# Project-Splinter/MonoPort

Measured on AMD Instinct MI355X. Metric: reconstructions/sec (512^2 in, 256^3 grid), higher is better.
Workload: dtype f32

## Files before the change

### monoport_amd/csrc/api.hip

```cpp
#include <cstdarg>
#include <cmath>
#include <cstring>

#include "mp_internal.h"
#include "encoder_kernels.h"
#include "octree_common.h"

namespace mp {

static thread_local std::string g_last_error;

int fail(mp_ctx *ctx, int code, const char *fmt, ...) {
  (void)ctx;
  char buf[512];
  va_list ap;
  va_start(ap, fmt);
  vsnprintf(buf, sizeof(buf), fmt, ap);
  va_end(ap);
  g_last_error = buf;
  return code;
}

int ensure_scratch(mp_ctx *ctx, hipStream_t st, size_t bytes, void **out) {
  mp_ctx::Arena &a = ctx->arenas[(void *)st];
// ... 2357 lines not shown
  DeviceGuard g(ctx->device);
  return launch_conv3x3_wino_pack(ctx, w, cout, cin, packed_wino, (hipStream_t)stream);
}

int mp_conv3x3_wino_supported(int cin, int cout, int h, int w) { return conv3x3_wino_supported(cin, cout, h, w) ? 1 : 0; }

int mp_conv3x3_pack16(mp_ctx *ctx, const float *w, int cout, int cin, void *packed16, float *wmax,
                      mp_stream stream) {
  if (!ctx) return MP_ERR_ARG;
  std::lock_guard<std::mutex> lk(ctx->mu);
  if (!w || !packed16 || !wmax || cout <= 0 || cin <= 0)
    return fail(ctx, MP_ERR_ARG, "mp_conv3x3_pack16: bad argument");
  if (cin % 16 || cout % 32)
    return fail(ctx, MP_ERR_UNSUPPORTED, "mp_conv3x3_pack16: needs Cin %% 16 == 0 and Cout %% 32 == 0");
  DeviceGuard g(ctx->device);
  return launch_conv3x3_pack16(ctx, w, cout, cin, packed16, wmax, (hipStream_t)stream);
}

int mp_conv3x3_gn16(mp_ctx *ctx, const float *x, int n, int cin, int h, int w, const float *ss, int relu,
                    int reflect, const void *packed16, const float *wmax, int cout, float *y, double *stats,
                    mp_stream stream) {
  if (!ctx) return MP_ERR_ARG;
  std::lock_guard<std::mutex> lk(ctx->mu);
  if (!x || !packed16 || !wmax || !y || n <= 0 || n > 65535 || cin <= 0 || cout <= 0 || h <= 0 || w <= 0)
    return fail(ctx, MP_ERR_ARG, "mp_conv3x3_gn16: bad argument");
  if (!aligned16(packed16)) return fail(ctx, MP_ERR_ARG, "mp_conv3x3_gn16: packed weights must be 16-byte aligned");
  DeviceGuard g(ctx->device);
  return launch_conv3x3_gn(ctx, x, n, cin, h, w, ss, relu, reflect, static_cast<const float *>(packed16),
                           wmax, cout, y, stats, (hipStream_t)stream);
}

int mp_conv1x1_pack(mp_ctx *ctx, const float *w1, int c1, const float *w2, int c2, int cout, int f16,
                    void *packed, float *wmax, mp_stream stream) {
  if (!ctx) return MP_ERR_ARG;
  std::lock_guard<std::mutex> lk(ctx->mu);
  if (!w1 || !packed || c1 <= 0 || c2 < 0 || (c2 > 0 && !w2) || (f16 && !wmax))
    return fail(ctx, MP_ERR_ARG, "mp_conv1x1_pack: bad argument");
  if (c1 % 64 || c2 % 64 || (cout != 128 && cout != 256))
    return fail(ctx, MP_ERR_UNSUPPORTED,
                "mp_conv1x1_pack: input channel counts must be multiples of 64, output channels 128 or 256");
  DeviceGuard g(ctx->device);
  return launch_conv1x1_pack(ctx, w1, c1, w2, c2, cout, f16, packed, wmax, (hipStream_t)stream);
}

int mp_conv1x1(mp_ctx *ctx, const float *x1, const float *ss1, int relu1, const float *x2, int n, int c1,
               int c2, int cout, int64_t hw, const void *packed, int f16, const float *wmax, const float *bias,
               const float *res, float *y, float *y_hwc, double *stats, mp_stream stream) {
  if (!ctx) return MP_ERR_ARG;
  std::lock_guard<std::mutex> lk(ctx->mu);
  if (!x1 || !packed || n <= 0 || hw <= 0 || (!y && !y_hwc) || (f16 && !wmax))
    return fail(ctx, MP_ERR_ARG, "mp_conv1x1: bad argument");
  if (!aligned16(packed) || (y_hwc && !aligned16(y_hwc)))
    return fail(ctx, MP_ERR_ARG, "mp_conv1x1: packed weights / y_hwc must be 16-byte aligned");
  DeviceGuard g(ctx->device);
  return launch_conv1x1_raw(ctx, x1, ss1, relu1, x2, n, c1, c2, cout, hw, packed, f16, wmax, bias, res, y,
                            y_hwc, stats, (hipStream_t)stream);
}

int mp_scale_shift_add(mp_ctx *ctx, const float *t, const float *ss, const float *res, int n, int c,
                       int64_t hw, float *y, mp_stream stream) {
  if (!ctx) return MP_ERR_ARG;
  std::lock_guard<std::mutex> lk(ctx->mu);
  if (!t || !ss || !res || !y || n <= 0 || c <= 0 || hw <= 0)
    return fail(ctx, MP_ERR_ARG, "mp_scale_shift_add: bad argument");
  if (hw % 4 || !aligned16(t) || !aligned16(res) || !aligned16(y))
    return fail(ctx, MP_ERR_UNSUPPORTED, "mp_scale_shift_add: needs HW %% 4 == 0 and 16-byte aligned buffers");
  DeviceGuard g(ctx->device);
  return launch_scale_shift_add(ctx, t, ss, res, (long long)n * c, hw, y, (hipStream_t)stream);
}

int mp_conv3x3_supported(int cin, int cout, int h, int w) { return conv3x3_supported(cin, cout, h, w) ? 1 : 0; }
int mp_conv_stats_supported(int cout) { return conv_stats_supported(cout) ? 1 : 0; }

int mp_gn_stat_slices(void) { return gn_stat_slices(); }

int mp_conv3x3_stat_slices(int cout, int n, int h, int w, int f16) {
  if (cout < 32 || cout % 32 || n < 1 || h < 1 || w < 32) return 0;
  return conv3x3_stat_slices(cout, n, h, w, f16 != 0);
}

void mp_query_tune(int small_tiles) { mp::query_small_set_gate(small_tiles); }

void mp_conv3x3_tune(int nr) {
  conv3x3_set_nr(nr & 0x1fff);
  conv1x1_set_mrw((nr >> 12) & 3);
}

int mp_conv3x3_gn(mp_ctx *ctx, const float *x, int n, int cin, int h, int w, const float *ss, int relu,
                  int reflect, const float *packed, int cout, float *y, double *stats, mp_stream stream) {
  if (!ctx) return MP_ERR_ARG;
  std::lock_guard<std::mutex> lk(ctx->mu);
  if (!x || !packed || !y || n <= 0 || n > 65535 || cin <= 0 || cout <= 0 || h <= 0 || w <= 0)
    return fail(ctx, MP_ERR_ARG, "mp_conv3x3_gn: bad argument");
  if (!aligned16(packed)) return fail(ctx, MP_ERR_ARG, "mp_conv3x3_gn: packed weights must be 16-byte aligned");
  DeviceGuard g(ctx->device);
  return launch_conv3x3_gn(ctx, x, n, cin, h, w, ss, relu, reflect, packed, nullptr, cout, y, stats,
                           (hipStream_t)stream);
}

int mp_gn_stats(mp_ctx *ctx, const float *x, int n, int c, int64_t hw, int groups, double *partial,
                mp_stream stream) {
  if (!ctx) return MP_ERR_ARG;
  std::lock_guard<std::mutex> lk(ctx->mu);
  if (!x || !partial || n <= 0 || c <= 0 || hw <= 0 || groups <= 0)
    return fail(ctx, MP_ERR_ARG, "mp_gn_stats: bad argument");
  if (c % groups || hw % 4 || !aligned16(x))
    return fail(ctx, MP_ERR_UNSUPPORTED, "mp_gn_stats: needs C %% groups == 0, HW %% 4 == 0, 16-byte aligned x");
  DeviceGuard g(ctx->device);
  return launch_gn_stats(ctx, x, n, c, hw, groups, partial, (hipStream_t)stream);
}

int mp_gn_finalize(mp_ctx *ctx, const double *partial, int n, int c, int groups, int slices,
                   int64_t count, const float *gamma, const float *beta, float eps, float *ss,
                   mp_stream stream) {
  if (!ctx) return MP_ERR_ARG;
  std::lock_guard<std::mutex> lk(ctx->mu);
  if (!partial || !gamma || !beta || !ss || n <= 0 || c <= 0 || groups <= 0 || slices <= 0 ||
      count <= 0 || c % groups || c / groups > 64)
    return fail(ctx, MP_ERR_ARG, "mp_gn_finalize: bad argument");
  DeviceGuard g(ctx->device);
  return launch_gn_finalize(ctx, partial, n, c, groups, slices, (double)count, gamma, beta, eps, ss,
                            (hipStream_t)stream);
}

static GnOut to_out(const mp_gn_out *f) {
  GnOut g = gn_out_none();
  if (!f) return g;
  g.acc = reinterpret_cast<long long *>(f->acc);
  g.partial = f->partial;
  return g;
}
static long long out_cap(const mp_gn_out *f) { return f && f->partial ? (long long)f->partial_doubles : -1; }
static GnIn to_in(const mp_gn_in *f) {
  GnIn g = gn_in_none();
  if (!f) return g;
  g.acc = reinterpret_cast<const long long *>(f->acc);
  g.gamma = f->gamma;
  g.beta = f->beta;
  g.eps = f->eps;
  g.ss = f->acc ? nullptr : f->ss;
  return g;
}

int mp_conv3x3_ex(mp_ctx *ctx, const mp_conv3x3_args *q, mp_stream stream) {
  if (!ctx) return MP_ERR_ARG;
  std::lock_guard<std::mutex> lk(ctx->mu);
  if (!q || !q->x || !q->packed || (!q->y && !q->y2) || q->n <= 0 || q->n > 65535 || q->cin <= 0 || q->cout <= 0 ||
      q->h <= 0 || q->w <= 0)
    return fail(ctx, MP_ERR_ARG, "mp_conv3x3_ex: bad argument");
  if (!aligned16(q->packed)) return fail(ctx, MP_ERR_ARG, "mp_conv3x3_ex: packed weights must be 16-byte aligned");
  DeviceGuard g(ctx->device);
  ConvArgs a;
  a.x = q->x;
  a.gn = to_in(&q->gn);
  a.wp = static_cast<const float *>(q->packed);
  a.y = q->y;
  a.y2 = q->y2;
  a.res = q->res;
  a.y2_c = q->y2 ? q->y2_channels : 32;
  a.y2_off = q->y2 ? q->y2_offset : 0;
  a.fin = to_out(&q->fin);
  a.fin2 = to_out(&q->fin2);
  a.n_img = q->n;
  a.cin = q->cin;
  a.cout = q->cout;
  a.h = q->h;
  a.w = q->w;
// ... 187 lines not shown
```

### monoport_amd/csrc/conv3x3.hip

```cpp
#include "mp_internal.h"
#include "query_common.h"
#include "gn_tail.h"

namespace mp {

constexpr int kCK = 16;
constexpr int kPixBytes = kCK * 4;
constexpr int kMaxCin = 512;
constexpr int kConvWps = 2;
constexpr int kTileW = 32;
constexpr int halo_pixels(int px) { return (px / kTileW + 2) * (kTileW + 2); }
constexpr int stage_iters(int px) { return (halo_pixels(px) + 63) / 64; }

__global__ void conv3x3_pack_kernel(const float *__restrict__ w, int cout, int cin,
                                    float *__restrict__ wp) {
  const long long total = (long long)cout * cin * 9;
  const int kgt = (cin / kCK) * 18;
  for (long long t = blockIdx.x * (long long)blockDim.x + threadIdx.x; t < total;
       t += (long long)gridDim.x * blockDim.x) {
    const int i = (int)(t & 3), lane = (int)((t >> 2) & 63);
    const long long q = t >> 8;
    const int kg = (int)(q % kgt), rb = (int)(q / kgt);
    const int g = kg & 1, tap = (kg >> 1) % 9, chunk = (kg >> 1) / 9;
    const int co = 32 * rb + (lane & 31);
// ... 669 lines not shown
#pragma unroll
  for (int n = 0; n < NR; ++n)
#pragma unroll
    for (int t = 0; t < 16; ++t) v[n][t] = acc[n][t] * inv_scale;
  conv_epilogue<32 * RBW, CW, NR, 16>(p, v, 0, img, tile, tiles, y0, x0, rbi, cwi, lane, smem);
}

__global__ __launch_bounds__(64) void gn_finalize_kernel(const double *__restrict__ partial, int groups,
                                                         int slices, double count, int cpg,
                                                         const float *__restrict__ gamma,
                                                         const float *__restrict__ beta, float eps,
                                                         float *__restrict__ ss) {
  const int g = blockIdx.x % groups, n = blockIdx.x / groups;
  const double *pp = partial + (long long)blockIdx.x * slices * 2;
  double a = 0.0, b = 0.0;
  for (int i = threadIdx.x; i < slices; i += 64) {
    a += pp[2 * i];
    b += pp[2 * i + 1];
  }
#pragma unroll
  for (int o = 32; o > 0; o >>= 1) {
    a += __shfl_xor(a, o);
    b += __shfl_xor(b, o);
  }
  const double mean_d = a / count;
  const double var_d = fmax(b / count - mean_d * mean_d, 0.0);
  const float mean = (float)mean_d;
  const float rstd = (float)(1.0 / sqrt(var_d + (double)eps));
  if ((int)threadIdx.x < cpg) {
    const int c = g * cpg + threadIdx.x;
    const float sc = rstd * gamma[c];
    float *o = ss + ((long long)n * groups * cpg + c) * 2;
    o[0] = sc;
    o[1] = beta[c] - mean * sc;
  }
}

__global__ __launch_bounds__(256) void scale_shift_add_kernel(const float *__restrict__ t,
                                                              const float *__restrict__ ss,
                                                              const float *__restrict__ res,
                                                              long long hw4, long long total4,
                                                              float *__restrict__ y) {
  const f32x4 *t4 = reinterpret_cast<const f32x4 *>(t), *r4 = reinterpret_cast<const f32x4 *>(res);
  f32x4 *y4 = reinterpret_cast<f32x4 *>(y);
  for (long long i = blockIdx.x * (long long)blockDim.x + threadIdx.x; i < total4;
       i += (long long)gridDim.x * blockDim.x) {
    const long long plane = i / hw4;
    const float sc = ss[2 * plane], sh = ss[2 * plane + 1];
    const f32x4 a = t4[i], r = r4[i];
    f32x4 o;
#pragma unroll
    for (int k = 0; k < 4; ++k) o[k] = r[k] + (a[k] * sc + sh);
    y4[i] = o;
  }
}

int launch_scale_shift_add(mp_ctx *ctx, const float *t, const float *ss, const float *res, long long planes,
                           long long hw, float *y, hipStream_t st) {
  const long long total4 = planes * (hw / 4);
  long long blocks = (total4 + 255) / 256;
  if (blocks > 16384) blocks = 16384;
  hipLaunchKernelGGL(scale_shift_add_kernel, dim3((unsigned)blocks), dim3(256), 0, st, t, ss, res, hw / 4,
                     total4, y);
  MP_HIP(ctx, hipGetLastError());
  return MP_OK;
}

int launch_conv3x3_pack(mp_ctx *ctx, const float *w, int cout, int cin, float *wp, hipStream_t st) {
  const long long total = (long long)cout * cin * 9;
  long long blocks = (total + 255) / 256;
  if (blocks > 4096) blocks = 4096;
  hipLaunchKernelGGL(conv3x3_pack_kernel, dim3((unsigned)blocks), dim3(256), 0, st, w, cout, cin, wp);
  MP_HIP(ctx, hipGetLastError());
  return MP_OK;
}

static int g_conv_nr = 0;
static int g_conv_sk = -1;

static int g_conv_wino = 1;
static long long g_conv_wino_min_wgs = 128;

void conv3x3_set_nr(int nr) {
  conv3x3_wino_set_variant((nr & 0x800) ? 64 : (nr & 0x1000) ? 128 : 0);
  nr &= ~0x1800;
  g_conv_nr = nr & 0xff;
  g_conv_wino = (nr >> 8) == 0 ? 1 : 0;
  nr &= ~0x400;
  g_conv_sk = (nr >> 8) == 0 ? -1 : (nr >> 8) - 1;
}

struct ConvPlan {
  int rbw, nr, tw, th, tiles;
  bool sk;
};

static ConvPlan conv_plan(int cout, int n, int h, int w, bool f16) {
  ConvPlan c;
  c.rbw = cout % 128 == 0 ? 4 : cout % 64 == 0 ? 2 : 1;
  const int cw = 4 / c.rbw;
  const long long pix = (long long)n * h * w;
  const long long wg1 = pix / (32 * cw) * (cout / (32 * c.rbw));
  const long long wg2 = wg1 / 2;
  c.nr = ((wg2 + 255) / 256) * 2 <= (wg1 + 255) / 256 ? 2 : 1;
  if (g_conv_nr > 0) c.nr = g_conv_nr;
  if (c.nr > 2 && (c.rbw == 1 || !f16)) c.nr = 2;
  c.sk = !f16 && (g_conv_sk >= 0 ? g_conv_sk == 1 : wg1 < 512);
  if (c.sk) {
    c.rbw = 1;
    c.nr = g_conv_nr > 0 ? (g_conv_nr > 2 ? 2 : g_conv_nr) : (pix / 64 * (cout / 32) >= 512 ? 2 : 1);
    if (h < c.nr) c.nr = 1;
    c.tw = kTileW;
    c.th = c.nr;
  } else {
    c.tw = kTileW;
    c.th = 32 * c.nr * cw / c.tw;
  }
  c.tiles = (h / c.th) * (w / c.tw);
  return c;
}

int conv3x3_stat_slices(int cout, int n, int h, int w, bool f16) { return conv_plan(cout, n, h, w, f16).tiles; }

bool conv3x3_supported(int cin, int cout, int h, int w) {
  return !(cin % kCK || cout % 32 || cin < kCK || cout < 32 || w < 32 || (w & (w - 1)) || h < 8 ||
           (h & (h - 1)));
}

bool conv_stats_supported(int cout) { return cout >= 32 && cout % 32 == 0 && 32 % (cout / 32) == 0; }

int launch_absmax(mp_ctx *ctx, const float *src, long long n, unsigned int *out_bits, hipStream_t st);

int launch_conv3x3_pack16(mp_ctx *ctx, const float *w, int cout, int cin, void *wp, float *wmax,
                          hipStream_t st) {
  const long long total = (long long)cout * cin * 9;
  int rc = launch_absmax(ctx, w, total, reinterpret_cast<unsigned int *>(wmax), st);
  if (rc != MP_OK) return rc;
  long long blocks = (total + 255) / 256;
  if (blocks > 4096) blocks = 4096;
  hipLaunchKernelGGL(conv3x3_pack16_kernel, dim3((unsigned)blocks), dim3(256), 0, st, w, cout, cin, wmax,
                     static_cast<_Float16 *>(wp));
  MP_HIP(ctx, hipGetLastError());
  return MP_OK;
}

template <int RBW, int NR>
static int launch_conv16_t(mp_ctx *ctx, const ConvArgs &a, const float *wmax, int tiles, hipStream_t st) {
  const int lds = 2 * (a.th + 2) * (a.tw + 2) * kPixBytes;
  auto kern = conv3x3_gn16_kernel<RBW, NR>;
  int rc = raise_lds_limit(ctx, reinterpret_cast<const void *>(kern), 2 * halo_pixels(32 * NR * (4 / RBW)) * kPixBytes);
  if (rc != MP_OK) return rc;
  hipLaunchKernelGGL(kern, dim3((unsigned)(tiles * a.n_img), (unsigned)(a.cout / (32 * RBW))), dim3(256),
                     lds, st, a, wmax);
  MP_HIP(ctx, hipGetLastError());
  return MP_OK;
}

template <int RBW, int NR>
static int launch_conv_t(mp_ctx *ctx, const ConvArgs &a, int tiles, hipStream_t st) {
  const int lds = 2 * (a.th + 2) * (a.tw + 2) * kPixBytes;
  auto kern = conv3x3_gn_kernel<RBW, NR>;
  int rc = raise_lds_limit(ctx, reinterpret_cast<const void *>(kern), 2 * halo_pixels(32 * NR * (4 / RBW)) * kPixBytes);
  if (rc != MP_OK) return rc;
  hipLaunchKernelGGL(kern, dim3((unsigned)(tiles * a.n_img), (unsigned)(a.cout / (32 * RBW))), dim3(256),
                     lds, st, a);
  MP_HIP(ctx, hipGetLastError());
  return MP_OK;
}
// ... 531 lines not shown
```

### monoport_amd/csrc/conv_wino.hip

```cpp
#include "mp_internal.h"
#include "query_common.h"
#include "gn_tail.h"

#pragma clang fp contract(off)

namespace mp {

constexpr int kWnThreads = 512;
constexpr int kWnTX = 8, kWnTY = 4;
constexpr int kWnPW = 2 * kWnTX + 2;
constexpr int kWnPH = 2 * kWnTY + 2;
constexpr int kWnPix = kWnPW * kWnPH;
constexpr int kWnPasses = (kWnPix + 63) / 64;
constexpr int kWnRow = 80;
constexpr int kWnRawBytes = kWnPix * kWnRow;
constexpr int kWnVBytes = 16 * 32 * kWnRow;
constexpr int kWnRaw = 0;
constexpr int kWnV = 2 * kWnRawBytes;
constexpr int kWnXchBytes = 8 * 2 * 2 * 4 * 64 * 16;
constexpr int kWnStat = kWnXchBytes;
constexpr int kWnLds = kWnStat + 8192;
constexpr int kWnAhead = 3;
static_assert(kWnV + 2 * kWnVBytes <= kWnXchBytes, "the exchange region covers the K loop's buffers");
static_assert(kWnLds <= 160 * 1024, "LDS");
// ... 464 lines not shown
    ring[i] = wload128(ws, a_base + ((cc >> 1) * 8 + i * 2 + (cc & 1)) * 64);
  };

  stage_load(0);
  GnAffine affine;
  gn_affine_load(p.gn, p.cin, affine);
  gn_load_stats(p.gn, img, gn_stats);
  a_load(0, 0);
  a_load(1, 0);
  __syncthreads();
  gn_table_fill(p.gn, img, p.cin, gn_stats, affine, ss_in);
  __syncthreads();
  stage_store(0);
  stage_load(1);
  __syncthreads();
  transform(0);
  stage_store(1);
  stage_load(2);
  __syncthreads();

#pragma unroll 1
  for (int chunk = 0; chunk < n_chunks; ++chunk) {
    const unsigned char *vb = smem + kW8V + (chunk & 1) * kW8VBytes + boff;
    const bool more1 = chunk + 1 < n_chunks;
    f32x4 b[2];
#pragma unroll
    for (int i = 0; i < 2; ++i) b[i] = *reinterpret_cast<const f32x4 *>(vb + i * 4 * 32 * kW8Row);
    a_load(2, chunk);
    a_load(3, chunk);
    if (more1 && rbh == 0) transform((chunk + 1) & 1);
    __builtin_amdgcn_sched_barrier(0);
#pragma unroll
    for (int ii = 0; ii < 4; ++ii)
#pragma unroll
      for (int i = 0; i < 2; ++i) acc[i] = __builtin_amdgcn_mfma_f32_32x32x2f32(ring[i][ii], b[i][ii], acc[i], 0, 0, 0);
    __builtin_amdgcn_sched_barrier(0);
#pragma unroll
    for (int i = 0; i < 2; ++i) b[i] = *reinterpret_cast<const f32x4 *>(vb + (i + 2) * 4 * 32 * kW8Row);
    a_load(0, chunk + 1);
    a_load(1, chunk + 1);
    stage_store(chunk & 1);
    stage_load(chunk + 3);
    __builtin_amdgcn_sched_barrier(0);
#pragma unroll
    for (int ii = 0; ii < 4; ++ii)
#pragma unroll
      for (int i = 2; i < 4; ++i) acc[i] = __builtin_amdgcn_mfma_f32_32x32x2f32(ring[i][ii], b[i - 2][ii], acc[i], 0, 0, 0);
    if (more1 && rbh == 1) transform((chunk + 1) & 1);
    __syncthreads();
  }

  f32x4 *xch = reinterpret_cast<f32x4 *>(smem);
#pragma unroll
  for (int q = 0; q < 4; ++q) {
    f32x4 s0, s1;
#pragma unroll
    for (int e = 0; e < 4; ++e) {
      const int t = 4 * q + e;
      s0[e] = (acc[0][t] + acc[1][t]) + acc[2][t];
      s1[e] = (acc[1][t] - acc[2][t]) - acc[3][t];
    }
    xch[((wv * 2 + 0) * 4 + q) * 64 + lane] = s0;
    xch[((wv * 2 + 1) * 4 + q) * 64 + lane] = s1;
  }
  const int r_o = jf & 1, qh = jf >> 1;
  WinoTail<NCH, 8> tail(p, 8 * qh, img, tile, y0, x0, rbh, r_o, lane);
  tail.load_res();
  __syncthreads();
  f32x2 pr[8];
#pragma unroll
  for (int qq = 0; qq < 2; ++qq) {
    f32x4 s[4];
#pragma unroll
    for (int j = 0; j < 4; ++j) s[j] = xch[(((4 * rbh + j) * 2 + r_o) * 4 + 2 * qh + qq) * 64 + lane];
#pragma unroll
    for (int e = 0; e < 4; ++e) {
      pr[4 * qq + e].x = (s[0][e] + s[1][e]) + s[2][e];
      pr[4 * qq + e].y = (s[1][e] - s[2][e]) - s[3][e];
    }
  }
  tail.finish(pr, smem + kW8Stat);
}

int launch_conv3x3_wino_pack(mp_ctx *ctx, const float *w, int cout, int cin, float *up, hipStream_t st) {
  const long long total = 16LL * cout * cin;
  long long blocks = (total + 255) / 256;
  if (blocks > 4096) blocks = 4096;
  hipLaunchKernelGGL(conv3x3_wino_pack_kernel, dim3((unsigned)blocks), dim3(256), 0, st, w, cout, cin, up);
  MP_HIP(ctx, hipGetLastError());
  return MP_OK;
}

bool conv3x3_wino_supported(int cin, int cout, int h, int w) {
  return cin % 16 == 0 && cin >= 16 && cin <= 512 && cout % 64 == 0 && h % (2 * kWnTY) == 0 && w % (2 * kWnTX) == 0;
}

int conv3x3_wino_tiles(int h, int w) { return (h / (2 * kWnTY)) * (w / (2 * kWnTX)); }

static int g_wino_variant = 0;
void conv3x3_wino_set_variant(int v) { g_wino_variant = v; }
bool conv3x3_wino_forced() { return g_wino_variant != 0; }
static bool wino_use64(const ConvArgs &a) {
  if (a.cout % 128) return true;
  if (g_wino_variant) return g_wino_variant == 64;
  return (long long)conv3x3_wino_tiles(a.h, a.w) * a.n_img * (a.cout / 128) < 2048;
}
long long conv3x3_wino_workgroups(const ConvArgs &a) {
  return (long long)conv3x3_wino_tiles(a.h, a.w) * a.n_img * (a.cout / (wino_use64(a) ? 64 : 128));
}

int launch_conv3x3_wino(mp_ctx *ctx, const ConvArgs &a, hipStream_t st) {
  if (gn_wanted(a.fin) && !conv_stats_supported(a.cout))
    return fail(ctx, MP_ERR_UNSUPPORTED,
                "conv3x3: statistics of y need Cout / 32 to divide 32 (Cout = 32, 64, 128, 256, 512, 1024); got %d", a.cout);
  const int tiles = conv3x3_wino_tiles(a.h, a.w);
  if (wino_use64(a)) {
    auto kern = conv3x3_wino64_kernel;
    if (const int rc = raise_lds_limit(ctx, reinterpret_cast<const void *>(kern), kW8Lds)) return rc;
    hipLaunchKernelGGL(kern, dim3((unsigned)(tiles * a.n_img), (unsigned)(a.cout / 64)), dim3(kWnThreads), kW8Lds, st, a);
  } else {
    auto kern = conv3x3_wino_kernel<2>;
    if (const int rc = raise_lds_limit(ctx, reinterpret_cast<const void *>(kern), kWnLds)) return rc;
    hipLaunchKernelGGL(kern, dim3((unsigned)(tiles * a.n_img), (unsigned)(a.cout / 128)), dim3(kWnThreads), kWnLds, st, a);
  }
  MP_HIP(ctx, hipGetLastError());
  return MP_OK;
}

}
```

### monoport_amd/ops.py

```python
import collections
import ctypes
import math
import os
import threading

import numpy as np
import torch

from . import _lib
from .synthetic import LAST_OP, MLP_DIMS

DIRECTIONS = {"front": 0, "back": 1, "left": 2, "right": 3}

_contexts = {}
_contexts_lock = threading.Lock()


class Context:

    def __init__(self, device_index):
        self.lib = _lib.load()
        assert self.lib.mp_max_frames() == MAX_FRAMES, "_lib.MAX_FRAMES and the library's kMaxFrames disagree"
        assert self.lib.mp_max_frame_views() == MAX_FRAME_VIEWS, "_lib.MAX_FRAME_VIEWS and MP_MAX_FRAME_VIEWS disagree"
        self.device_index = int(device_index)
# ... 2301 lines not shown
CONNECTIVITIES = (_lib.CONN_6, _lib.CONN_26)


def _keep_largest(who, sdfs, level, connectivity, fill, gates, out):
    vols, n, r, dev = _one_size_volumes(who, sdfs)
    if connectivity not in CONNECTIVITIES:
        raise ValueError("%s: connectivity must be one of %s, got %r" % (who, list(CONNECTIVITIES), connectivity))
    if not float(fill) <= float(level):
        raise ValueError("%s: fill %r would be foreground at level %r" % (who, fill, level))
    _gates(who, gates, n, dev)
    cleaned, stats = (None, None) if out is None else out
    if cleaned is None:
        cleaned = torch.empty((n, r, r, r), dtype=torch.float32, device=dev).unbind(0)
    else:
        cleaned = _frame_rows(who, "out[0] (volumes)", cleaned, n, (r, r, r), torch.float32, dev)
    if stats is None:
        stats = torch.empty((n, 4), dtype=torch.int32, device=dev).unbind(0)
    else:
        stats = _frame_rows(who, "out[1] (stats)", stats, n, (4,), torch.int32, dev)
    ctx = get_context(dev)
    for f0, f1 in _frame_chunks(n):
        ctx.check(ctx.lib.mp_volume_keep_largest_batch(
            ctx.handle, f1 - f0, _ptr_array(vols[f0:f1]), r, float(level), int(connectivity), float(fill),
            _ptr_array(cleaned[f0:f1]), _ptr_array(stats[f0:f1]),
            None if gates is None else _ptr_array(gates[f0:f1]), _stream(vols[0])), "mp_volume_keep_largest_batch")
    _keep_until_done(dev, vols, gates)
    return list(zip(cleaned, stats))


def keep_largest_raw(sdf, level=0.5, connectivity=6, fill=0.0, out=None):
    return _keep_largest("keep_largest_raw", [sdf], level, connectivity, fill, None,
                         None if out is None else ([out], None))[0]


def keep_largest_raw_batch(sdfs, level=0.5, connectivity=6, fill=0.0, gates=None, out=None):
    return _keep_largest("keep_largest_raw_batch", sdfs, level, connectivity, fill, gates, out)


def group_norm(x, groups, weight, bias, eps=1e-5, relu=False):
    ctx = get_encoder_context(x.device)
    n, c = x.shape[0], x.shape[1]
    hw = x.shape[2] * x.shape[3]
    y = torch.empty_like(x)
    ctx.check(ctx.lib.mp_group_norm(ctx.handle, _ptr(x), n, c, hw, int(groups), _ptr(weight),
                                    _ptr(bias), float(eps), int(bool(relu)), _ptr(y), _stream(x)),
              "mp_group_norm")
    return y


def group_norm_supported(x):
    return (x.is_cuda and x.dim() == 4 and x.dtype == torch.float32
            and x.is_contiguous() and (x.shape[2] * x.shape[3]) % 4 == 0)


def upsample_bicubic2x(x, add=None):
    ctx = get_encoder_context(x.device)
    n, c, h, w = x.shape
    y = torch.empty((n, c, 2 * h, 2 * w), dtype=torch.float32, device=x.device)
    ctx.check(ctx.lib.mp_upsample_bicubic2x(ctx.handle, _ptr(x), n * c, h, w,
                                            _ptr(add) if add is not None else None, _ptr(y),
                                            _stream(x)), "mp_upsample_bicubic2x")
    return y


def concat3_add_supported(a, b, c, shortcut):
    ts = (a, b, c, shortcut)
    return (all(t.is_cuda and t.dtype == torch.float32 and t.dim() == 4 for t in ts)
            and (a.shape[2] * a.shape[3]) % 4 == 0
            and a.shape[1] + b.shape[1] + c.shape[1] == shortcut.shape[1])


def concat3_add(a, b, c, shortcut):
    a, b, c, shortcut = _f32c(a), _f32c(b), _f32c(c), _f32c(shortcut)
    ctx = get_encoder_context(a.device)
    n, ca, h, w = a.shape
    y = torch.empty_like(shortcut)
    ctx.check(ctx.lib.mp_concat3_add(ctx.handle, _ptr(a), ca, _ptr(b), b.shape[1], _ptr(c),
                                     c.shape[1], _ptr(shortcut), n, h * w, _ptr(y), _stream(a)),
              "mp_concat3_add")
    return y


CONV_WINOGRAD = os.environ.get("MONOPORT_CONV_WINOGRAD", "1") != "0"


class PackedConv3x3:

    def __init__(self, weight, precision="f32"):
        w = _f32c(weight.detach())
        self.cout, self.cin = int(w.shape[0]), int(w.shape[1])
        if tuple(w.shape[2:]) != (3, 3):
            raise ValueError("PackedConv3x3 wants a [Cout,Cin,3,3] weight, got %s" % (tuple(w.shape),))
        if precision not in ("f32", "f16x3"):
            raise ValueError("conv precision must be 'f32' or 'f16x3'")
        self.precision = precision
        ctx = get_encoder_context(w.device)
        self.data = torch.empty((w.numel(),), dtype=torch.float32, device=w.device)
        self.wmax = None
        self.wino = None
        if precision == "f32":
            ctx.check(ctx.lib.mp_conv3x3_pack(ctx.handle, _ptr(w), self.cout, self.cin, _ptr(self.data),
                                              _stream(w)), "mp_conv3x3_pack")
            if CONV_WINOGRAD and self.cout % 64 == 0:
                self.wino = torch.empty((16 * self.cout * self.cin,), dtype=torch.float32, device=w.device)
                ctx.check(ctx.lib.mp_conv3x3_pack_wino(ctx.handle, _ptr(w), self.cout, self.cin, _ptr(self.wino),
                                                       _stream(w)), "mp_conv3x3_pack_wino")
        else:
            self.wmax = torch.zeros((1,), dtype=torch.float32, device=w.device)
            ctx.check(ctx.lib.mp_conv3x3_pack16(ctx.handle, _ptr(w), self.cout, self.cin, _ptr(self.data),
                                                _ptr(self.wmax), _stream(w)), "mp_conv3x3_pack16")
        w.record_stream(torch.cuda.current_stream(w.device))


def conv3x3_supported(cin, cout, h, w):
    return bool(_lib.load().mp_conv3x3_supported(int(cin), int(cout), int(h), int(w)))


def conv3x3_stats_supported(cout):
    return bool(_lib.load().mp_conv_stats_supported(int(cout)))


def scale_shift_add(t, ss, res):
    ctx = get_encoder_context(t.device)
    t, res = t.contiguous(), res.contiguous()
    n, c = t.shape[0], t.shape[1]
    y = torch.empty_like(t)
    ctx.check(ctx.lib.mp_scale_shift_add(ctx.handle, _ptr(t), _ptr(ss), _ptr(res), n, c,
                                         t.shape[2] * t.shape[3], _ptr(y), _stream(t)), "mp_scale_shift_add")
    return y


def conv3x3_gn(x, ss, packed, relu=True, want_stats=False, reflect=False):
    ctx = get_encoder_context(x.device)
    n, cin, h, w = x.shape
    if cin != packed.cin:
        raise ValueError("conv3x3_gn: input has %d channels, weights expect %d" % (cin, packed.cin))
    y = torch.empty((n, packed.cout, h, w), dtype=torch.float32, device=x.device)
    stats = None
    if want_stats:
        s = ctx.lib.mp_conv3x3_stat_slices(packed.cout, n, h, w, int(packed.precision == "f16x3"))
        stats = (torch.empty((n, 32, s, 2), dtype=torch.float64, device=x.device), s)
    if packed.precision == "f32":
        ctx.check(ctx.lib.mp_conv3x3_gn(ctx.handle, _ptr(x), n, cin, h, w,
                                        _ptr(ss) if ss is not None else None, int(bool(relu)),
                                        int(bool(reflect)), _ptr(packed.data), packed.cout, _ptr(y),
                                        _ptr(stats[0]) if stats else None, _stream(x)), "mp_conv3x3_gn")
    else:
        ctx.check(ctx.lib.mp_conv3x3_gn16(ctx.handle, _ptr(x), n, cin, h, w,
                                          _ptr(ss) if ss is not None else None, int(bool(relu)),
                                          int(bool(reflect)), _ptr(packed.data), _ptr(packed.wmax),
                                          packed.cout, _ptr(y),
                                          _ptr(stats[0]) if stats else None, _stream(x)),
                  "mp_conv3x3_gn16")
    return y, stats


class PackedConv1x1:

    def __init__(self, w1, b1=None, w2=None, b2=None, precision="f32"):
        w1 = _f32c(w1.detach().reshape(w1.shape[0], -1))
        self.cout = int(w1.shape[0])
        if self.cout not in (128, 256):
            raise ValueError("conv1x1 is built for 128 or 256 output channels, got %d" % self.cout)
        self.c1, self.c2 = int(w1.shape[1]), 0
        if w2 is not None:
            w2 = _f32c(w2.detach().reshape(w2.shape[0], -1))
# ... 356 lines not shown
```

Before: 220.4.

## Add Winograd conv kernel that transforms input tiles in registers for small Cin

Adds a new Winograd F(2,3) 3x3 convolution kernel that keeps the raw input patch in LDS with a padded layout. Each wave computes the input transform on the fly in registers, interleaved with MFMA accumulation, instead of staging pre-transformed V tiles. It is selected by default when Cin is at most 64 and the 64-wide variant would be used, and a tune bit can force it. The aim is to cut LDS traffic and footprint so that more workgroups fit per CU on shallow layers, at the cost of repeating transform arithmetic across waves.

New measurement: 220.7 (median of 6 runs). No clear change (+0.1%).

```diff
diff --git a/monoport_amd/csrc/api.hip b/monoport_amd/csrc/api.hip
--- a/monoport_amd/csrc/api.hip
+++ b/monoport_amd/csrc/api.hip
@@ -2463,7 +2463,7 @@
 void mp_query_tune(int small_tiles) { mp::query_small_set_gate(small_tiles); }
 
 void mp_conv3x3_tune(int nr) {
-  conv3x3_set_nr(nr & 0x1fff);
+  conv3x3_set_nr(nr & 0x5fff);
   conv1x1_set_mrw((nr >> 12) & 3);
 }
 
diff --git a/monoport_amd/csrc/conv3x3.hip b/monoport_amd/csrc/conv3x3.hip
--- a/monoport_amd/csrc/conv3x3.hip
+++ b/monoport_amd/csrc/conv3x3.hip
@@ -775,8 +775,8 @@
 static long long g_conv_wino_min_wgs = 128;
 
 void conv3x3_set_nr(int nr) {
-  conv3x3_wino_set_variant((nr & 0x800) ? 64 : (nr & 0x1000) ? 128 : 0);
-  nr &= ~0x1800;
+  conv3x3_wino_set_variant((nr & 0x4000) ? 1 : (nr & 0x800) ? 64 : (nr & 0x1000) ? 128 : 0);
+  nr &= ~0x5800;
   g_conv_nr = nr & 0xff;
   g_conv_wino = (nr >> 8) == 0 ? 1 : 0;
   nr &= ~0x400;
diff --git a/monoport_amd/csrc/conv_wino.hip b/monoport_amd/csrc/conv_wino.hip
--- a/monoport_amd/csrc/conv_wino.hip
+++ b/monoport_amd/csrc/conv_wino.hip
@@ -570,6 +570,209 @@
   tail.finish(pr, smem + kW8Stat);
 }
 
+constexpr int kRkRowU = 9 * 33;
+constexpr int kRkRawBytes = (9 * kRkRowU + 4 * 6 + 17 * 16 + 8 + 16) * 16;
+constexpr int kRkStat = kW8XchBytes;
+constexpr int kRkLds = kRkStat + 4096;
+static_assert(kRkRawBytes <= kW8XchBytes, "the exchange region covers the raw patch");
+static_assert(2 * (kRkLds + 4608) <= 160 * 1024, "two workgroups per CU");
+__host__ __device__ constexpr int rk_pix_unit(int pr, int pc) { return pr * kRkRowU + (pr >> 1) * 6 + pc * 16 + (pc >> 1); }
+
+__global__ __launch_bounds__(kWnThreads, 4) void conv3x3_wino_rk_kernel(ConvArgs p) {
+  constexpr int NCH = 64;
+  extern __shared__ __attribute__((aligned(16))) unsigned char smem[];
+  const int tid = threadIdx.x;
+  const int lane = tid & 63;
+  const int wv = __builtin_amdgcn_readfirstlane(tid >> 6);
+  const int jl = lane & 31, h = lane >> 5;
+  const int jf = wv & 3, rbh = wv >> 2;
+
+  const int tiles_x = p.w / (2 * kWnTX), tiles = tiles_x * (p.h / (2 * kWnTY));
+  const int tile = blockIdx.x % tiles, img = blockIdx.x / tiles;
+  const int y0 = (tile / tiles_x) * (2 * kWnTY), x0 = (tile % tiles_x) * (2 * kWnTX);
+  const int hw = p.h * p.w;
+  const int n_chunks = p.cin / 8;
+
+  const WStream ws = make_wstream(p.wpw, p.wpw_floats, lane);
+  __shared__ float gn_stats[64];
+  __shared__ __attribute__((aligned(16))) float ss_in[2 * 512];
+
+  const __amdgpu_buffer_rsrc_t rs_x = __builtin_amdgcn_make_buffer_rsrc(
+      const_cast<float *>(p.x + (long long)img * p.cin * hw), 0, p.cin * hw * 4, 0x00020000);
+  auto stage_load = [&](float (&stg)[8], int it, int half, int ln) {
+    const int lp = ln + 64 * it;
+    const int r = lp / kWnPW, c = lp - r * kWnPW;
+    int gy = y0 - 1 + r, gx = x0 - 1 + c;
+    bool ok = lp < kWnPix;
+    if (p.reflect) {
+      gy = gy < 0 ? -gy : (gy >= p.h ? 2 * p.h - 2 - gy : gy);
+      gx = gx < 0 ? -gx : (gx >= p.w ? 2 * p.w - 2 - gx : gx);
+    } else {
+      ok = ok && gy >= 0 && gy < p.h && gx >= 0 && gx < p.w;
+    }
+    const int o = ok ? (gy * p.w + gx) * 4 : 0;
+#pragma unroll
+    for (int k = 0; k < 8; ++k)
+      stg[k] = __builtin_bit_cast(float, __builtin_amdgcn_raw_buffer_load_b32(rs_x, o, min(64 * half + 8 * wv + k, p.cin - 1) * hw * 4, 0));
+  };
+  auto stage_store = [&](const float (&stg)[8], int it, int half, int ln) {
+    const int lp = ln + 64 * it;
+    if (64 * half + 8 * wv < p.cin && lp < kWnPix) {
+      const f32x4 *ssv = reinterpret_cast<const f32x4 *>(ss_in + 2 * (64 * half + 8 * wv));
+      const int r = lp / kWnPW, c = lp - r * kWnPW;
+      const int gy = y0 - 1 + r, gx = x0 - 1 + c;
+      const bool pad = !p.reflect && (gy < 0 || gy >= p.h || gx < 0 || gx >= p.w);
+      f32x4 *dst = reinterpret_cast<f32x4 *>(smem + rk_pix_unit(r, c) * 16 + wv * 32);
+#pragma unroll
+      for (int q = 0; q < 2; ++q) {
+        const f32x4 ss[2] = {ssv[2 * q], ssv[2 * q + 1]};
+        f32x4 v;
+#pragma unroll
+        for (int k = 0; k < 4; ++k) {
+          float t = fmaf(stg[4 * q + k], ss[k >> 1][2 * (k & 1)], ss[k >> 1][2 * (k & 1) + 1]);
+          if (p.relu) t = fmaxf(t, 0.0f);
+          v[k] = pad ? 0.0f : t;
+        }
+        dst[q] = v;
+      }
+    }
+  };
+
+  const int ca = jf == 0 ? 0 : jf == 2 ? 2 : 1;
+  const int cb = jf == 0 ? 2 : jf == 1 ? 2 : jf == 2 ? 1 : 3;
+  const float sg = jf == 1 ? 1.0f : -1.0f;
+  const int lbase = ((jl >> 3) * 600 + (jl & 7) * 33 + h) * 16;
+  const unsigned char *ra = smem + lbase + (ca * 16 + (ca >> 1)) * 16;
+  const unsigned char *rb = smem + lbase + (cb * 16 + (cb >> 1)) * 16;
+  f32x4 ta[2], tb[2];
+  auto rows_read = [&](int r0, int cofs) {
+#pragma unroll
+    for (int r = 0; r < 2; ++r) {
+      const int ro = ((r0 + r) * kRkRowU + ((r0 + r) >> 1) * 6) * 16;
+      ta[r] = *reinterpret_cast<const f32x4 *>(ra + ro + cofs);
+      tb[r] = *reinterpret_cast<const f32x4 *>(rb + ro + cofs);
+    }
+  };
+  auto rows_t = [&](f32x4 &t0, f32x4 &t1) {
+    t0 = __builtin_elementwise_fma(tb[0], (f32x4)sg, ta[0]);
+    t1 = __builtin_elementwise_fma(tb[1], (f32x4)sg, ta[1]);
+  };
+  auto rows_v = [&](f32x4 (&v)[4], const f32x4 (&t)[4]) {
+    v[0] = pk_sub4(t[0], t[2]);
+    v[1] = t[1] + t[2];
+    v[2] = pk_sub4(t[2], t[1]);
+    v[3] = pk_sub4(t[1], t[3]);
+  };
+
+  const int a_base = ((((int)blockIdx.y * 2 + rbh) * 4 + jf) * (p.cin / 16)) * 8 * 64;
+  f32x16 acc[4];
+#pragma unroll
+  for (int i = 0; i < 4; ++i)
+#pragma unroll
+    for (int t = 0; t < 16; ++t) acc[i][t] = 0.0f;
+  f32x4 ring[4];
+  auto a_load = [&](int i, int c) {
+    const int cc = min(c, n_chunks - 1);
+    ring[i] = wload128(ws, a_base + ((cc >> 1) * 8 + i * 2 + (cc & 1)) * 64);
+  };
+
+  float stg[kWnPasses][8];
+#pragma unroll
+  for (int it = 0; it < kWnPasses; ++it) stage_load(stg[it], it, 0, lane);
+  GnAffine affine;
+  gn_affine_load(p.gn, p.cin, affine);
+  gn_load_stats(p.gn, img, gn_stats);
+  a_load(0, 0);
+  a_load(1, 0);
+  __syncthreads();
+  gn_table_fill(p.gn, img, p.cin, gn_stats, affine, ss_in);
+  __syncthreads();
+#pragma unroll
+  for (int it = 0; it < kWnPasses; ++it) stage_store(stg[it], it, 0, lane);
+  __syncthreads();
+
+#pragma unroll 1
+  for (int c0 = 0; c0 < n_chunks; c0 += 8) {
+    if (c0) {
+      int ln = lane;
+      asm volatile("" : "+v"(ln));
+      float s0[8], s1[8];
+      stage_load(s0, 0, c0 >> 3, ln);
+      stage_load(s1, 1, c0 >> 3, ln);
+      __syncthreads();
+      stage_store(s0, 0, c0 >> 3, ln);
+      stage_load(s0, 2, c0 >> 3, ln);
+      stage_store(s1, 1, c0 >> 3, ln);
+      stage_store(s0, 2, c0 >> 3, ln);
+      __syncthreads();
+    }
+    const int c1 = min(c0 + 8, n_chunks);
+    f32x4 v[4], t[4];
+    rows_read(0, 0);
+    rows_t(t[0], t[1]);
+    rows_read(2, 0);
+    rows_t(t[2], t[3]);
+    rows_v(v, t);
+#pragma unroll 1
+    for (int chunk = c0; chunk < c1; ++chunk) {
+      const int cofs = (min(chunk + 1, c1 - 1) - c0) * 32;
+      a_load(2, chunk);
+      a_load(3, chunk);
+      rows_read(0, cofs);
+      __builtin_amdgcn_sched_barrier(0);
+#pragma unroll
+      for (int ii = 0; ii < 4; ++ii)
+#pragma unroll
+        for (int i = 0; i < 2; ++i) acc[i] = __builtin_amdgcn_mfma_f32_32x32x2f32(ring[i][ii], v[i][ii], acc[i], 0, 0, 0);
+      __builtin_amdgcn_sched_barrier(0);
+      rows_t(t[0], t[1]);
+      rows_read(2, cofs);
+      a_load(0, chunk + 1);
+      a_load(1, chunk + 1);
+      __builtin_amdgcn_sched_barrier(0);
+#pragma unroll
+      for (int ii = 0; ii < 4; ++ii)
+#pragma unroll
+        for (int i = 2; i < 4; ++i) acc[i] = __builtin_amdgcn_mfma_f32_32x32x2f32(ring[i][ii], v[i][ii], acc[i], 0, 0, 0);
+      __builtin_amdgcn_sched_barrier(0);
+      rows_t(t[2], t[3]);
+      rows_v(v, t);
+    }
+  }
+  __syncthreads();
+
+  f32x4 *xch = reinterpret_cast<f32x4 *>(smem);
+#pragma unroll
+  for (int q = 0; q < 4; ++q) {
+    f32x4 s0, s1;
+#pragma unroll
+    for (int e = 0; e < 4; ++e) {
+      const int t = 4 * q + e;
+      s0[e] = (acc[0][t] + acc[1][t]) + acc[2][t];
+      s1[e] = (acc[1][t] - acc[2][t]) - acc[3][t];
+    }
+    xch[((wv * 2 + 0) * 4 + q) * 64 + lane] = s0;
+    xch[((wv * 2 + 1) * 4 + q) * 64 + lane] = s1;
+  }
+  const int r_o = jf & 1, qh = jf >> 1;
+  WinoTail<NCH, 8> tail(p, 8 * qh, img, tile, y0, x0, rbh, r_o, lane);
+  tail.load_res();
+  __syncthreads();
+  f32x2 pr[8];
+#pragma unroll
+  for (int qq = 0; qq < 2; ++qq) {
+    f32x4 s[4];
+#pragma unroll
+    for (int j = 0; j < 4; ++j) s[j] = xch[(((4 * rbh + j) * 2 + r_o) * 4 + 2 * qh + qq) * 64 + lane];
+#pragma unroll
+    for (int e = 0; e < 4; ++e) {
+      pr[4 * qq + e].x = (s[0][e] + s[1][e]) + s[2][e];
+      pr[4 * qq + e].y = (s[1][e] - s[2][e]) - s[3][e];
+    }
+  }
+  tail.finish(pr, smem + kRkStat);
+}
+
 int launch_conv3x3_wino_pack(mp_ctx *ctx, const float *w, int cout, int cin, float *up, hipStream_t st) {
   const long long total = 16LL * cout * cin;
   long long blocks = (total + 255) / 256;
@@ -585,16 +788,22 @@
 
 int conv3x3_wino_tiles(int h, int w) { return (h / (2 * kWnTY)) * (w / (2 * kWnTX)); }
 
+constexpr int kWinoRk = 1;
 static int g_wino_variant = 0;
 void conv3x3_wino_set_variant(int v) { g_wino_variant = v; }
 bool conv3x3_wino_forced() { return g_wino_variant != 0; }
 static bool wino_use64(const ConvArgs &a) {
   if (a.cout % 128) return true;
-  if (g_wino_variant) return g_wino_variant == 64;
+  if (g_wino_variant) return g_wino_variant != 128;
   return (long long)conv3x3_wino_tiles(a.h, a.w) * a.n_img * (a.cout / 128) < 2048;
 }
+static bool wino_use_rk(const ConvArgs &a) {
+  if (a.cin > 128) return false;
+  if (g_wino_variant) return g_wino_variant == kWinoRk;
+  return a.cin <= 64 && wino_use64(a);
+}
 long long conv3x3_wino_workgroups(const ConvArgs &a) {
-  return (long long)conv3x3_wino_tiles(a.h, a.w) * a.n_img * (a.cout / (wino_use64(a) ? 64 : 128));
+  return (long long)conv3x3_wino_tiles(a.h, a.w) * a.n_img * (a.cout / (wino_use_rk(a) || wino_use64(a) ? 64 : 128));
 }
 
 int launch_conv3x3_wino(mp_ctx *ctx, const ConvArgs &a, hipStream_t st) {
@@ -602,7 +811,11 @@
     return fail(ctx, MP_ERR_UNSUPPORTED,
                 "conv3x3: statistics of y need Cout / 32 to divide 32 (Cout = 32, 64, 128, 256, 512, 1024); got %d", a.cout);
   const int tiles = conv3x3_wino_tiles(a.h, a.w);
-  if (wino_use64(a)) {
+  if (wino_use_rk(a)) {
+    auto kern = conv3x3_wino_rk_kernel;
+    if (const int rc = raise_lds_limit(ctx, reinterpret_cast<const void *>(kern), kRkLds)) return rc;
+    hipLaunchKernelGGL(kern, dim3((unsigned)(tiles * a.n_img), (unsigned)(a.cout / 64)), dim3(kWnThreads), kRkLds, st, a);
+  } else if (wino_use64(a)) {
     auto kern = conv3x3_wino64_kernel;
     if (const int rc = raise_lds_limit(ctx, reinterpret_cast<const void *>(kern), kW8Lds)) return rc;
     hipLaunchKernelGGL(kern, dim3((unsigned)(tiles * a.n_img), (unsigned)(a.cout / 64)), dim3(kWnThreads), kW8Lds, st, a);
diff --git a/monoport_amd/ops.py b/monoport_amd/ops.py
--- a/monoport_amd/ops.py
+++ b/monoport_amd/ops.py
@@ -2407,6 +2407,7 @@
 
 
 CONV_WINOGRAD = os.environ.get("MONOPORT_CONV_WINOGRAD", "1") != "0"
+CONV3X3_TUNE_WINO_RK = 0x4000
 
 
 class PackedConv3x3:
```
